# yixuan/ADMM

Measured on AMD Instinct MI355X. Metric: ADMM iterations/sec, Lasso tall n=100000 p=10000 (100-lambda warm-started path), higher is better.
Workload: dtype f32; 1 GPU; admm_lasso tall path (BASELINE configs[1]); n=100000, p=10000, nlambda=100, standardize=True, intercept=True, parallelism=single GPU, step=one cold-started warm-chained lambda path

## Files before the change

admm_amd/csrc/lasso_tall.hip:

```cpp
#include "prep.h"
#include "gemv_kernels.h"
#include "symv_kernels.h"
#include "solvers.h"
#include "sgl_host.h"
#include "box_host.h"
#include "comm.h"
#include "loop_driver.h"
#include "plan_host.h"
#include "peer_device.h"
#include "probe.h"

namespace admm {

struct TallCtl {
    double rho, lam, eps_primal, eps_dual, adj_a, adj_c, tau;
    double a_next, tau_next;
    int mode;
    int restart;
    int iter;
    int lam_idx;
    int done;
    int first;
    int total;
    int fin_idx;
    int fin_niter;
    int pad;
};

struct TallParams {
    int p, nwg, nseg, maxit, nlam, enet;
    long long part_stride;
    double eps_abs, eps_rel, alpha, sqrt_p;
    const double* lambdas;
    const float* XY;
    const float* a_part; const float* b_part;
    const float* dot0; const float* dot1; const float* axp0; const float* axp1;
    long long ldo; int nrb, p32; SymvSched sched;
    float* x; float* z0; float* z1; float* y0; float* y1; float* adj_z; float* adj_y; float* u; float* w;
    TallCtl* ctl;
    double* P;
    float* beta;
    int* niter;
    int* done_host;
#ifdef ADMM_HIP_PROBE
    long long* probe;
#endif
    double* trace;
    long long trace_cap;
    const float* refine_ab;
    long long refine_ld;
    float* state;
    long long state_cap;
    unsigned long long* verdict;
    unsigned long long run_tag;
};

__host__ __device__ inline unsigned long long tall_verdict_word(unsigned long long run_tag, int total, bool discard) {
    return run_tag | ((unsigned long long)(unsigned)total << 1) | (discard ? 1ull : 0ull);
}
constexpr int kVerdictShift = 33;
constexpr int kVerdictWords = kSyVerdictReplicas * kSyVerdictStride;

constexpr int kTailThreads = 256;
constexpr int kTailLanes = kSySumLanes;
constexpr int kTailElems = kTailThreads / kTailLanes;

__device__ __forceinline__ double tall_load_partial(const double* p, bool in_launch) {
    if (!in_launch) return *p;
    return __longlong_as_double((long long)__hip_atomic_load(reinterpret_cast<const unsigned long long*>(p), __ATOMIC_RELAXED, __HIP_MEMORY_SCOPE_AGENT));
}
__device__ __forceinline__ void tall_store_wt(float* p, float v) {
    __hip_atomic_store(reinterpret_cast<unsigned int*>(p), __float_as_uint(v), __ATOMIC_RELAXED, __HIP_MEMORY_SCOPE_AGENT);
}
__device__ __forceinline__ void tall_store_wt(double* p, double v) {
    __hip_atomic_store(reinterpret_cast<unsigned long long*>(p), (unsigned long long)__double_as_longlong(v), __ATOMIC_RELAXED, __HIP_MEMORY_SCOPE_AGENT);
}

template <bool IN_LAUNCH = false>
__device__ void tall_decide(const TallParams& q, int par) {
    __shared__ double dscratch[6 * (kTailThreads / 64)];
    WIDE_PROBE_DECL
    WIDE_PROBE(0);
    const TallCtl in = q.ctl[par];
    TallCtl* outp = &q.ctl[par ^ 1];
    if (in.done) {
        if (threadIdx.x == 0) { TallCtl o = in; o.fin_idx = -1; *outp = o; }
        return;
    }
    WIDE_PROBE(1);
    double acc[6] = {0, 0, 0, 0, 0, 0};
    const double* Pin = q.P + (size_t)par * q.nwg * 8;
    for (int w = threadIdx.x; w < q.nwg; w += kTailThreads) {
#pragma unroll
        for (int k = 0; k < 6; ++k) acc[k] += tall_load_partial(Pin + (size_t)w * 8 + k, IN_LAUNCH);
    }
    block_sum<double, 6>(acc, dscratch);
    if (threadIdx.x != 0) return;
    WIDE_PROBE(2);
    const double r2 = acc[0], dz2 = acc[1], daz2 = acc[2], x2 = acc[3], z2 = acc[4], y2 = acc[5];
    double tr_rp = 0, tr_rd = 0, tr_c = 0, tr_code = ADMM_TRACE_COLD;
    TallCtl out = in;
    out.first = 0;
    out.fin_idx = -1; out.fin_niter = 0;
    if (!in.first) {
        const double rp = sqrt(r2);
        const double rd = in.rho * sqrt(dz2);
        tr_rp = rp; tr_rd = rd;
        if (rp < in.eps_primal && rd < in.eps_dual) {
            out.fin_idx = in.lam_idx; out.fin_niter = in.iter + 1;
            out.mode = 0;
            tr_code = ADMM_TRACE_CONVERGED;
        } else {
            const double old_c = in.adj_c;
            const double c = in.rho * rp * rp + in.rho * daz2;
            tr_c = c;
            if (c < 0.999 * old_c) {
                out.adj_a = in.a_next; out.adj_c = c; out.tau = in.tau_next; out.restart = 0;
                tr_code = ADMM_TRACE_ACCELERATE;
            } else {
                out.adj_a = 1.0; out.adj_c = old_c / 0.999; out.tau = -1.0; out.restart = 1;
                tr_code = ADMM_TRACE_RESTART;
            }
            out.mode = 1;
            out.iter = in.iter + 1;
            if (in.iter + 1 >= q.maxit) {
                out.fin_idx = in.lam_idx; out.fin_niter = q.maxit + 1;
            }
        }
        if (out.fin_idx >= 0) {
            out.lam_idx = in.lam_idx + 1;
            out.iter = 0;
            if (out.lam_idx >= q.nlam) out.done = 1;
            else out.lam = q.lambdas[out.lam_idx];
            q.niter[out.fin_idx] = out.fin_niter;
        }
    } else {
        out.mode = 1; out.tau = 0.0; out.restart = 0;
    }
    if (q.verdict != nullptr && (out.mode == 0 || out.done)) {
        const unsigned long long word = tall_verdict_word(q.run_tag, in.total + 1, true);
        for (int r = 0; r < kSyVerdictReplicas; ++r)
            __hip_atomic_store(q.verdict + (size_t)r * kSyVerdictStride, word, __ATOMIC_RELAXED, __HIP_MEMORY_SCOPE_AGENT);
    }
    out.eps_primal = fmax(sqrt(x2), sqrt(z2)) * q.eps_rel + q.sqrt_p * q.eps_abs;
    out.eps_dual = sqrt(y2) * q.eps_rel + q.sqrt_p * q.eps_abs;
    out.a_next = 0.5 + 0.5 * sqrt(1.0 + 4.0 * out.adj_a * out.adj_a);
    out.tau_next = (out.adj_a - 1.0) / out.a_next;
    out.total = in.total + 1;
    *outp = out;
    if (out.done) *q.done_host = 1;
    WIDE_PROBE(3);
    WIDE_PROBE_FLUSH(2, in.total);
    if (q.trace != nullptr && in.total < q.trace_cap) {
        double* t = q.trace + (size_t)in.total * ADMM_TRACE_FIELDS;
        t[0] = in.lam_idx; t[1] = in.iter; t[2] = in.eps_primal; t[3] = in.eps_dual; t[4] = tr_rp; t[5] = tr_rd;
        t[6] = tr_c; t[7] = in.adj_c; t[8] = tr_code; t[9] = in.rho; t[10] = in.rho; t[11] = in.lam;
    }
}

struct TallDecideExtra {
    static constexpr bool kHas = true;
    TallParams q; int par;
    __device__ void operator()() const { tall_decide<false>(q, par); }
};

__device__ __forceinline__ float tall_extrapolate(float t1, float t, float cur, float old) {
#pragma clang fp contract(off)
    const float a = t1 * cur;
    const float b = t * old;
    return a - b;
}

struct TallElem { float zc, yc, zo, yo, adjz, adjy, x, xy; };

__device__ __forceinline__ TallElem tall_load_elem(const TallParams& q, int par, int i) {
    const float* zc_ = par ? q.z1 : q.z0; const float* yc_ = par ? q.y1 : q.y0;
    const float* zo_ = par ? q.z0 : q.z1; const float* yo_ = par ? q.y0 : q.y1;
    TallElem e;
    e.zc = zc_[i]; e.yc = yc_[i]; e.zo = zo_[i]; e.yo = yo_[i]; e.adjz = q.adj_z[i]; e.adjy = q.adj_y[i]; e.x = q.x[i]; e.xy = q.XY[i];
    return e;
}

__device__ __forceinline__ float tall_soft(float vec, double pen) {
    const double v = (double)vec;
    return v > pen ? (float)(v - pen) : (v < -pen ? (float)(v + pen) : 0.f);
}

__device__ __forceinline__ double tall_block_shrink(double nrm2, double pen) {
    const double nrm = sqrt(nrm2);
    return nrm > pen ? 1.0 - pen / nrm : 0.0;
}

template <bool WT = false>
__device__ __forceinline__ void tall_update_elem(const TallParams& q, const TallCtl& c, int par, int i, const TallElem& e, float a, float b, double (&acc)[6]) {
#pragma clang fp contract(off)
    float* zo_ = par ? q.z0 : q.z1; float* yo_ = par ? q.y0 : q.y1;
    const float zc = e.zc, yc = e.yc, zo = e.zo, yo = e.yo;
    if (c.fin_idx >= 0) q.beta[(size_t)c.fin_idx * q.p + i] = zc;
    if (c.done) return;
    float adjz, adjy, x;
    if (c.mode) {
        if (c.restart) { adjz = zo; adjy = yo; x = b; }
        else {
            const float t = (float)c.tau, t1 = (float)(1.0 + c.tau);
            adjz = tall_extrapolate(t1, t, zc, zo);
            adjy = tall_extrapolate(t1, t, yc, yo);
            x = a;
        }
    } else { adjz = e.adjz; adjy = e.adjy; x = e.x; }
    const float rho_f = (float)c.rho;
    const float vec = x + adjy / rho_f;
    const double pen = c.lam / c.rho;
    float zn;
    if (!q.enet) zn = tall_soft(vec, pen);
    else {
        const float thresh = (float)(q.alpha * pen);
        const float denom = (float)(1.0 + pen * (1.0 - q.alpha));
        zn = vec > thresh ? (vec - thresh) / denom : (vec < -thresh ? (vec + thresh) / denom : 0.f);
    }
    const float r = x - zn;
    const float yn = adjy + rho_f * r;
    const float dz = zn - zc, daz = zn - adjz;
    acc[0] = (double)r * r; acc[1] = (double)dz * dz; acc[2] = (double)daz * daz;
    acc[3] = (double)x * x; acc[4] = (double)zn * zn; acc[5] = (double)yn * yn;
    q.x[i] = x; zo_[i] = zn; yo_[i] = yn; q.adj_z[i] = adjz; q.adj_y[i] = adjy;
    if (q.state != nullptr && c.total < q.state_cap) {
        float* s = q.state + (size_t)c.total * 5 * q.p;
        s[i] = x; s[q.p + i] = zn; s[2 * (size_t)q.p + i] = yn; s[3 * (size_t)q.p + i] = adjz; s[4 * (size_t)q.p + i] = adjy;
    }
    const float tn = (float)c.tau_next, tn1 = (float)(1.0 + c.tau_next);
    const float adjz_a = tall_extrapolate(tn1, tn, zn, zc), adjy_a = tall_extrapolate(tn1, tn, yn, yc);
    const float un = (float)((double)(e.xy - adjy_a) + c.rho * (double)adjz_a);
    const float wn = (float)((double)(e.xy - yc) + c.rho * (double)zc);
    if (WT) { tall_store_wt(q.u + i, un); tall_store_wt(q.w + i, wn); }
    else { q.u[i] = un; q.w[i] = wn; }
}

__device__ __forceinline__ void tall_publish_norms(const TallParams& q, int par, const double (&acc)[6], double* scratch) {
    static_assert(kTailLanes == 8, "owner lanes are the multiples of 8");
    const int lane = threadIdx.x & 63, wid = threadIdx.x >> 6;
    const double v8[8] = {acc[0], acc[1], acc[2], acc[3], acc[4], acc[5], 0.0, 0.0};
    const double tot = halving_sum8_top(v8, lane);
    if ((lane & 7) == 0 && lane < 48) scratch[(lane >> 3) * (kTailThreads / 64) + wid] = tot;
    __syncthreads();
    if (threadIdx.x < 6) {
// ... 522 lines not shown
            free_b += pool_cached_bytes();
            if (opt_set(Opt::TEST_FREE_BYTES)) free_b = (size_t)opt_int(Opt::TEST_FREE_BYTES, 0);
            const bool have_gram = d.gram.get() && d.ldgram == ldp;
            const bool inv64_wanted = p < 4096 || opt_is(Opt::INVERSE, "f64");
            const double mat = (double)ldp * (double)ldp * 4.0;
            const double need = (have_gram ? 0.0 : mat) + (inv64_wanted ? 2.0 * mat : 0.5 * mat) + (opt_on(Opt::REFINE) ? mat : 0.0) +
                                (shard && ci.nranks > 1 ? mat + mat / ci.nranks : 0.0) +
                                (mt ? mt_partial_floats() * 4.0 : 0.0);
            if (need > 0.97 * (double)free_b) {
                char msg[320];
                std::snprintf(msg, sizeof msg, "tall solver: the cached %d x %d inverse and its workspace need %.1f GB, the device has %.1f GB free; "
                              "use $parallel() (row blocks, admm_hip_parlasso) or fewer columns", p, p, need / 1e9, (double)free_b / 1e9);
                throw Error(ADMM_ERR_MEMORY, msg);
            }
        }
        double t0 = now_s();
        const bool gram_given = d.gram.get() && d.ldgram == ldp;
        if (gram_given) {
            M = std::move(d.gram);
            S.t_gram = d.t_gram_tail;
        } else {
            M.alloc((size_t)ldp * ldp); M.zero(st);
            gram_full<float>(d.X.get(), d.ldx, n, p, true, M.get(), ldp, st);
            comm_stream_sync(st);
            S.t_gram = now_s() - t0;
        }
        bool inv64 = p < 4096;
        if (opt_set(Opt::INVERSE)) inv64 = opt_is(Opt::INVERSE, "f64");
        bool dist_factor = shard && ci.nranks > 1 && !inv64 && (p + 127) / 128 >= 2 * ci.nranks && p >= 256;
        if (opt_off(Opt::DIST_FACTOR)) dist_factor = false;

        rho = pb.opts.rho;
        t0 = now_s();
        if (rho <= 0) {
            SymMatVec<float> op(M.get(), ldp, p, st);
            int nmatop = 0;
            DevBuf<float> wsum;
            if (shard && ci.nranks > 1) wsum.alloc(ldp);
            const float ev = lanczos_largest_f32([&](const float* v, float* w_) {
                op(v, w_);
                if (shard && ci.nranks > 1) {
                    ADMM_HIP_CHECK(hipMemcpyAsync(wsum.get(), w_, (size_t)p * sizeof(float), hipMemcpyHostToDevice, st));
                    allreduce_sum_f32(wsum.get(), (size_t)p, st);
                    ADMM_HIP_CHECK(hipMemcpyAsync(w_, wsum.get(), (size_t)p * sizeof(float), hipMemcpyDeviceToHost, st));
                    comm_stream_sync(st);
                    comm_check();
                }
            }, p, &nmatop);
            S.eig_est = ev;
            rho = std::pow((double)ev, 1.0 / 3) * std::pow(lam_int[0], 2.0 / 3);
        }
        S.rho = rho;
        S.t_eigs = now_s() - t0;

        if (shard && ci.nranks > 1 && !gram_given) {
            const double tr0 = now_s();
            if (dist_factor) {
                const int nb128 = (p + 127) / 128, N = ci.nranks;
                const int nown = (nb128 + N - 1) / N;
                const size_t blk = (size_t)128 * ldp, cnt = (size_t)nown * blk;
                DevBuf<float> send((size_t)N * cnt), recv(cnt);
                send.zero(st);
                for (int k = 0; k < nb128; ++k) {
                    const size_t cols = (size_t)std::min(128, (int)ldp - k * 128);
                    ADMM_HIP_CHECK(hipMemcpyAsync(send.get() + ((size_t)(k % N) * nown + k / N) * blk, M.get() + (size_t)k * blk, cols * ldp * sizeof(float),
                                                  hipMemcpyDeviceToDevice, st));
                }
                reduce_scatter_sum_f32(send.get(), recv.get(), cnt, st);
                for (int k = ci.rank; k < nb128; k += N) {
                    const size_t cols = (size_t)std::min(128, (int)ldp - k * 128);
                    ADMM_HIP_CHECK(hipMemcpyAsync(M.get() + (size_t)k * blk, recv.get() + (size_t)(k / N) * blk, cols * ldp * sizeof(float), hipMemcpyDeviceToDevice, st));
                }
            } else {
                allreduce_sum_f32(M.get(), (size_t)ldp * ldp, st);
            }
            comm_stream_sync(st);
            comm_check();
            S.t_gram += now_s() - tr0;
        }

        refine = opt_on(Opt::REFINE) && !shard;
        if (refine) {
            Mg.alloc((size_t)ldp * ldp);
            ADMM_HIP_CHECK(hipMemcpyAsync(Mg.get(), M.get(), (size_t)ldp * ldp * sizeof(float), hipMemcpyDeviceToDevice, st));
            add_diag<float>(Mg.get(), ldp, p, (float)rho, st);
        }
        t0 = now_s();
        if (inv64) {
            spd_inverse_f32_via_f64(M.get(), ldp, p, (double)(float)rho, st);
        } else if (dist_factor) {
            add_diag<float>(M.get(), ldp, p, (float)rho, st);
            sy.init(p, st, ci.rank, ci.nranks);
            std::vector<int> need;
            {
                const int nb128 = (p + 127) / 128;
                std::vector<char> mark((size_t)nb128 * nb128, 0);
                for (const int4& t : sy.htiles)
                    for (int bi = 2 * t.x; bi <= 2 * t.x + 1 && bi < nb128; ++bi)
                        for (int bj = t.y / 128; bj <= (t.y + t.z - 1) / 128 && bj < nb128; ++bj)
                            if (bj <= bi && !mark[(size_t)bi * nb128 + bj]) { mark[(size_t)bi * nb128 + bj] = 1; need.push_back(bi << 16 | bj); }
            }
            double fl = 0;
            spd_inverse_mfma_f32_dist(M.get(), ldp, p, need, &fl, st);
            dist_flops = fl;
        } else {
            add_diag<float>(M.get(), ldp, p, (float)rho, st);
            spd_inverse_f32(M.get(), ldp, p, st);
        }
        comm_stream_sync(st);
        S.t_factor = now_s() - t0;
        d.X.release();

        use_sym = p >= 2048;
        if (opt_set(Opt::XUPDATE)) use_sym = opt_is(Opt::XUPDATE, "sym");
        if (refine) use_sym = true;
        if (shard) use_sym = true;
        if (mt) use_sym = true;
        pl = plan_gemv_t<float>(p, p, 2, 4);
        nwg = (p + kTailElems - 1) / kTailElems;
        if (grouped) nwg = pack_group_tiles();
        ldv = round_up(p, 256);
        if (use_sym) sy.init(p, st, shard ? ci.rank : 0, shard ? ci.nranks : 1);
        if (refine) {
            rab.alloc((size_t)2 * ldv); rab.zero(st);
            ruw.alloc((size_t)2 * ldv); ruw.zero(st);
            dD0.alloc((size_t)sy.nrb * sy.ldo); dD1.alloc((size_t)sy.nrb * sy.ldo);
            xD0.alloc((size_t)sy.nax_rows * sy.ldo); xD1.alloc((size_t)sy.nax_rows * sy.ldo);
            dD0.zero(st); dD1.zero(st); xD0.zero(st); xD1.zero(st);
        }
        if (shard) { ab.alloc((size_t)2 * ldp); ab.zero(st); }
        else if (!use_sym) { a_part.alloc((size_t)pl.nseg * ldp); b_part.alloc((size_t)pl.nseg * ldp); a_part.zero(st); b_part.zero(st); }
        const ExchangeForm xf = peer_exchange_form(shard, ci, reinterpret_cast<const void*>(tall_tail_kernel<TAIL_PEER1>), kTailThreads, nwg);
        peer_fused = xf.fused; peer_one = xf.one; exchange_code = xf.variant;
        const size_t npl = (size_t)std::max(mt, 1);
        x.alloc(npl * ldv); z0.alloc(npl * ldv); z1.alloc(npl * ldv); y0.alloc(npl * ldv); y1.alloc(npl * ldv);
        adj_z.alloc(npl * ldv); adj_y.alloc(npl * ldv); u.alloc(ldv); w.alloc(ldv);
        beta.alloc((size_t)nlam * p * npl); niter.alloc(nlam);
        P.alloc((size_t)2 * nwg * 8); dlam.alloc(nlam); ctl.alloc(2);
        u.zero(st); w.zero(st);
        ADMM_HIP_CHECK(hipMemcpyAsync(dlam.get(), lam_int.data(), nlam * sizeof(double), hipMemcpyHostToDevice, st));

        q.p = p; q.nwg = nwg; q.nseg = pl.nseg; q.maxit = pb.opts.maxit; q.nlam = nlam; q.enet = pb.enet ? 1 : 0;
        q.part_stride = ldp;
        q.eps_abs = pb.opts.eps_abs; q.eps_rel = pb.opts.eps_rel; q.alpha = (double)(float)pb.alpha; q.sqrt_p = std::sqrt((double)p * (double)npl);
        q.lambdas = dlam.get(); q.XY = XY.get(); q.a_part = a_part.get(); q.b_part = b_part.get();
        if (shard) { q.a_part = ab.get(); q.b_part = ab.get() + ldp; q.nseg = 1; }
        q.dot0 = sy.dot0.get(); q.dot1 = sy.dot1.get(); q.axp0 = sy.axp0.get(); q.axp1 = sy.axp1.get();
        q.ldo = sy.ldo; q.nrb = sy.nrb; q.p32 = sy.p32; q.sched = sy.sched;
        q.refine_ab = refine ? rab.get() : nullptr; q.refine_ld = ldv;
        q.x = x.get(); q.z0 = z0.get(); q.z1 = z1.get(); q.y0 = y0.get(); q.y1 = y1.get();
        q.adj_z = adj_z.get(); q.adj_y = adj_y.get(); q.u = u.get(); q.w = w.get();
        q.ctl = ctl.get(); q.P = P.get(); q.beta = beta.get(); q.niter = niter.get();
        q.done_host = hflag.p;
        verdict_on = use_sym && !shard && !refine && !mt && !opt_off(Opt::SYMV_VERDICT);
        verdict_mid = opt_int(Opt::SYMV_VERDICT, 2) == 2;
        if (verdict_on) {
            verdict.alloc(kVerdictWords + kSyVerdictStride); verdict.zero(st);
            q.verdict = verdict.get();
        }
#ifdef ADMM_HIP_PROBE
        probe.alloc((size_t)4096 * 4 * 8); probe.zero(st);
        q.probe = probe.get();
        sy.probe = probe.get();
#endif

        if (mt) {
            static const int kAutoRhs[kMtMax] = {2, 4, 8, 8, 12, 12, 8, 8, 4, 4, 12, 12, 4, 4, 8, 8};
            mt_rhs = kAutoRhs[mt - 1];
            if (const OptValue* v = opt(Opt::MT_RHS)) { if (v->i > 0) mt_rhs = kSyNR[v->i - 1]; }
            uw.alloc((size_t)2 * mt * ldv); uw.zero(st);
            const size_t ds = (size_t)sy.nrb * sy.ldo, as = (size_t)sy.nax_rows * sy.ldo;
            mdot.alloc((size_t)2 * mt * ds); maxp.alloc((size_t)2 * mt * as);
            mdot.zero(st); maxp.zero(st);
            x.zero(st); z0.zero(st); z1.zero(st); y0.zero(st); y1.zero(st); adj_z.zero(st); adj_y.zero(st);
            roww.alloc(p);
            ADMM_HIP_CHECK(hipMemcpyAsync(roww.get(), pb.row_weight.data(), (size_t)p * sizeof(double), hipMemcpyHostToDevice, st));
            mq.m = mt; mq.ldv = ldv; mq.ldxy = ldp; mq.uw = uw.get();
            mq.dot = mdot.get(); mq.axp = maxp.get(); mq.dot_stride = (long long)ds; mq.axp_stride = (long long)as;
            mq.row_w = roww.get();
        }
        ADMM_HIP_CHECK(hipHostMalloc(reinterpret_cast<void**>(&hbeta), (size_t)nlam * p * npl * sizeof(float), hipHostMallocDefault));
        comm_stream_sync(st);
    }

    float box_plan_lambda0() {
        std::vector<float> lo(p), hi(p), h(p);
        for (int j = 0; j < p; ++j) {
            lo[j] = box_round_lower(box_to_std(pb.box_lower[j], (double)d.scaleX[j], (double)d.scaleY));
            hi[j] = box_round_upper(box_to_std(pb.box_upper[j], (double)d.scaleX[j], (double)d.scaleY));
        }
        clamp.set(pb.box_lower, pb.box_upper);
        bpf.alloc((size_t)p); blo.alloc((size_t)p); bhi.alloc((size_t)p);
        ADMM_HIP_CHECK(hipMemcpyAsync(bpf.get(), pb.penalty_factor.data(), (size_t)p * sizeof(double), hipMemcpyHostToDevice, st));
        ADMM_HIP_CHECK(hipMemcpyAsync(blo.get(), lo.data(), (size_t)p * sizeof(float), hipMemcpyHostToDevice, st));
        ADMM_HIP_CHECK(hipMemcpyAsync(bhi.get(), hi.data(), (size_t)p * sizeof(float), hipMemcpyHostToDevice, st));
        read_back(h.data(), XY.get(), (size_t)p * sizeof(float), st);
        bq.pf = bpf.get(); bq.lo = blo.get(); bq.hi = bhi.get();
        return box_lambda0(h.data(), p, lo.data(), hi.data(), pb.penalty_factor.data());
    }

    float mt_lambda0() {
        std::vector<float> h((size_t)mt * ldp);
        read_back(h.data(), XY.get(), h.size() * sizeof(float), st);
        double best = 0.0;
        for (int j = 0; j < p; ++j) {
            if (!(pb.row_weight[j] > 0)) continue;
            double s2 = 0.0;
            for (int k = 0; k < mt; ++k) { const double v = (double)h[(size_t)k * ldp + j]; s2 += v * v; }
            best = std::max(best, std::sqrt(s2) / pb.row_weight[j]);
        }
        return (float)best;
    }
    double mt_partial_floats() const {
        const double nrb = (double)((p + kSyRB - 1) / kSyRB), ldo = nrb * kSyRB;
        return 2.0 * mt * (nrb + (double)((p + 31) / 32)) * ldo;
    }

    float group_lambda0() {
        std::vector<float> h(p);
        read_back(h.data(), XY.get(), (size_t)p * sizeof(float), st);
        double best = 0.0;
        for (size_t g = 0; g + 1 < pb.group_start.size(); ++g) {
            if (!(pb.group_weight[g] > 0)) continue;
            double s2 = 0.0;
            for (int j = pb.group_start[g]; j < pb.group_start[g + 1]; ++j) s2 += (double)h[j] * (double)h[j];
            best = std::max(best, std::sqrt(s2) / pb.group_weight[g]);
        }
        return (float)best;
    }

    float sgl_plan_lambda0() {
        std::vector<float> h(p);
        read_back(h.data(), XY.get(), (size_t)p * sizeof(float), st);
        return sgl_lambda0(h.data(), pb.group_start, pb.l1_weight, pb.group_weight);
    }

    int pack_group_tiles() {
        std::vector<int2> tiles;
        std::vector<GroupCoord> coord(p);
        const bool flat = pb.sgl && std::none_of(pb.group_weight.begin(), pb.group_weight.end(), [](double w) { return w > 0; });
        std::vector<int> each;
        if (flat) for (int j = 0; j <= p; ++j) each.push_back(j);
        const std::vector<int>& start = flat ? each : pb.group_start;
        int first = 0, count = 0;
        const auto flush = [&] { if (count > 0) tiles.push_back(make_int2(first, count)); first += count; count = 0; };
        for (size_t g = 0; g + 1 < start.size(); ++g) {
            const int gs = start[g], gn = start[g + 1] - gs;
            const double wg = flat ? 0.0 : pb.group_weight[g];
            ADMM_REQUIRE(gn >= 1 && gn <= kGroupMax && gs == first + count, "internal: bad group partition");
            for (int j = gs; j < gs + gn; ++j)
                coord[j] = GroupCoord{gs, gn, pb.sgl && gn == 1 ? sgl_single_weight(pb.l1_weight[j], wg) : wg};
            if (count + gn > kTailElems) flush();
            count += gn;
            if (gn > kTailElems) flush();
        }
        flush();
        gtiles.alloc(tiles.size()); gcoord.alloc(coord.size());
        ADMM_HIP_CHECK(hipMemcpyAsync(gtiles.get(), tiles.data(), tiles.size() * sizeof(int2), hipMemcpyHostToDevice, st));
        ADMM_HIP_CHECK(hipMemcpyAsync(gcoord.get(), coord.data(), coord.size() * sizeof(GroupCoord), hipMemcpyHostToDevice, st));
        if (pb.sgl) {
            gl1.alloc((size_t)p);
            ADMM_HIP_CHECK(hipMemcpyAsync(gl1.get(), pb.l1_weight.data(), (size_t)p * sizeof(double), hipMemcpyHostToDevice, st));
        }
        comm_stream_sync(st);
        gq.tiles = gtiles.get(); gq.coord = gcoord.get(); gq.l1 = pb.sgl ? gl1.get() : nullptr;
        return (int)tiles.size();
    }

    Records records() override { return {st, 5ll * p * std::max(mt, 1), &q.trace, &q.trace_cap, &q.state, &q.state_cap}; }

    void read_system(float* out, long long ld) override {
        if (!refine) throw Error(ADMM_ERR_INVALID_ARG, "the system matrix is only kept with ADMM_HIP_REFINE=1");
        ADMM_REQUIRE(out != nullptr && ld >= p, "bad output for the system matrix");
        ADMM_HIP_CHECK(hipMemcpy2D(out, (size_t)ld * sizeof(float), Mg.get(), (size_t)ldp * sizeof(float), (size_t)p * sizeof(float), (size_t)p, hipMemcpyDeviceToHost));
    }

    void run(LassoResult& res) override {
        admm_stats S = setup_stats;
        S.xupdate_variant = shard ? 2 : (use_sym ? 1 : 0);
        S.exchange_variant = exchange_code;
        S.refine = refine ? 1 : 0;
        S.factor_flops = dist_flops;
        res.lambda = lam_user;
        beta.zero(st); niter.zero(st);
        q.run_tag = ++run_no << kVerdictShift;
        const int init_n = std::max(p, 2 * nwg * 8);
        for (int k = 0; k < std::max(mt, 1); ++k) {
            TallParams qk = q;
            if (mt) {
                const size_t o = (size_t)k * ldv;
                qk.x += o; qk.z0 += o; qk.z1 += o; qk.y0 += o; qk.y1 += o; qk.adj_z += o; qk.adj_y += o;
                qk.XY += (size_t)k * ldp; qk.u = uw.get() + (size_t)(2 * k) * ldv; qk.w = uw.get() + (size_t)(2 * k + 1) * ldv;
            }
            hipLaunchKernelGGL(tall_init_kernel, dim3((init_n + 255) / 256), dim3(256), 0, st, qk, rho, lam_int[0]);
        }
        if (q.state != nullptr && mt)
            ADMM_HIP_CHECK(hipMemcpy2DAsync(q.state, (size_t)p * sizeof(float), XY.get(), (size_t)ldp * sizeof(float), (size_t)p * sizeof(float),
                                            (size_t)mt, hipMemcpyDeviceToDevice, st));
        else if (q.state != nullptr)
            ADMM_HIP_CHECK(hipMemcpyAsync(q.state, XY.get(), (size_t)p * sizeof(float), hipMemcpyDeviceToDevice, st));
        *hflag.p = 0;
#ifdef ADMM_HIP_PROBE
        sy.probe_idx = 0;
#endif

        const int batch = batch_iters(pb.batch_iters, 32);
        const int stride = pb.profile_stride;
        size_t nev = 0;
        const auto done_at = [&](long long g) -> const int* { return &ctl.get()[(int)(g & 1)].done; };
        const LoopTimes lt = run_until_done(st, done_at, batch, (long long)nlam * ((long long)pb.opts.maxit + 2) + 4, [&](long long g) {
            const int par = (int)(g & 1);
            const bool sample = stride > 0 && (g % stride) == stride / 2 && nev < 8192;
            hipEvent_t e0 = nullptr, e1 = nullptr;
            if (sample) {
                while (ev_pool.size() < nev + 2) {
                    hipEvent_t e; ADMM_HIP_CHECK(hipEventCreate(&e));
                    ev_pool.push_back(e);
                }
                e0 = ev_pool[nev]; e1 = ev_pool[nev + 1];
                nev += 2;
            }
            const TallDecideExtra dec{q, par};
            SymvVerdict vd;
            if (verdict_on) { vd.words = verdict.get(); vd.discard = tall_verdict_word(q.run_tag, (int)(g + 1), true); vd.early = verdict.get() + kVerdictWords; vd.mid = verdict_mid; }
            const int* skip = &ctl.get()[par].done;
            const auto xupdate = [&] {
                if (use_sym) sy.launch(M.get(), ldp, u.get(), w.get(), skip, st, dec, e0, e1, vd);
                else launch_gemv_t<float, 2, 4, TallDecideExtra>(pl, M.get(), ldp, p, p, u.get(), w.get(), a_part.get(), b_part.get(), ldp, skip, st, dec, e0, e1);
            };
            const auto group_tail = [&] {
                void (*tail)(TallParams, int, GroupTailParams) =
                    use_sym ? (pb.sgl ? tall_group_tail_kernel<TAIL_SYMV, true> : tall_group_tail_kernel<TAIL_SYMV>)
                            : (pb.sgl ? tall_group_tail_kernel<TAIL_GEMV, true> : tall_group_tail_kernel<TAIL_GEMV>);
                hipLaunchKernelGGL(tail, dim3(nwg), dim3(kTailThreads), 0, st, q, par, gq);
            };
            if (mt) {
                const int nvec = 2 * mt;
                for (int r0 = 0; r0 < nvec; r0 += mt_rhs) {
                    SymvNArgs a;
                    a.A = M.get(); a.lda = ldp; a.p = p;
                    a.v = uw.get() + (size_t)r0 * ldv; a.vstride = ldv;
                    a.dot = mdot.get() + (size_t)r0 * mq.dot_stride; a.dot_stride = mq.dot_stride;
                    a.axp = maxp.get() + (size_t)r0 * mq.axp_stride; a.axp_stride = mq.axp_stride;
                    a.nvec = std::min(mt_rhs, nvec - r0); a.ldo = sy.ldo; a.tiles = sy.tiles.get(); a.skip = skip;
                    hipEvent_t es = r0 == 0 ? e0 : nullptr, ee = r0 + mt_rhs >= nvec ? e1 : nullptr;
                    if (r0 == 0) symvn_launch(sy, mt_rhs, a, st, dec, es, ee);
                    else symvn_launch(sy, mt_rhs, a, st, SymvNoExtra(), es, ee);
                }
                hipLaunchKernelGGL(tall_mt_tail_kernel, dim3(nwg), dim3(kTailThreads), 0, st, q, par, mq);
            } else if (grouped) {
                xupdate();
                group_tail();
            } else if (shard && peer_fused) {
                sy.launch(M.get(), ldp, u.get(), w.get(), skip, st, dec, e0, e1);
                const PeerExchange ex = comm_peer_begin((size_t)2 * ldp * sizeof(float));
                if (peer_one) {
                    hipLaunchKernelGGL(tall_tail_kernel<TAIL_PEER1>, dim3(nwg), dim3(kTailThreads), 0, st, q, par, ex);
                } else {
                    hipLaunchKernelGGL(tall_shard_push_kernel, dim3(nwg), dim3(kTailThreads), 0, st, q, ex, ldp, skip);
                    hipLaunchKernelGGL(tall_tail_kernel<TAIL_PEER>, dim3(nwg), dim3(kTailThreads), 0, st, q, par, ex);
                }
            } else if (shard) {
                sy.launch(M.get(), ldp, u.get(), w.get(), skip, st, dec, e0, e1);
                hipLaunchKernelGGL(tall_shard_reduce_kernel, dim3(nwg), dim3(kTailThreads), 0, st, q, ab.get(), ldp, skip);
                allreduce_sum_f32(ab.get(), (size_t)2 * ldp, st);
                hipLaunchKernelGGL(tall_tail_kernel<TAIL_GEMV>, dim3(nwg), dim3(kTailThreads), 0, st, q, par, PeerExchange{});
            } else if (use_sym && refine) {
                sy.launch(M.get(), ldp, u.get(), w.get(), skip, st, dec, e0, e1);
                hipLaunchKernelGGL(tall_shard_reduce_kernel, dim3(nwg), dim3(kTailThreads), 0, st, q, rab.get(), ldv, skip);
                SymvArgsD ad;
                ad.A = Mg.get(); ad.lda = ldp; ad.p = p; ad.v0 = rab.get(); ad.v1 = rab.get() + ldv;
                ad.dot0 = dD0.get(); ad.dot1 = dD1.get(); ad.axp0 = xD0.get(); ad.axp1 = xD1.get(); ad.ldo = sy.ldo; ad.tiles = sy.tiles.get(); ad.skip = skip;
                hipLaunchKernelGGL(symv2_lower_f64acc_kernel, dim3(sy.ntiles), dim3(kSyThreads), 0, st, ad);
                hipLaunchKernelGGL(tall_refine_resid_kernel, dim3(nwg), dim3(kTailThreads), 0, st, q, dD0.get(), dD1.get(), xD0.get(), xD1.get(),
                                   ruw.get(), ruw.get() + ldv, skip);
                sy.launch(M.get(), ldp, ruw.get(), ruw.get() + ldv, skip, st, SymvNoExtra());
                hipLaunchKernelGGL(tall_tail_kernel<TAIL_SYMV>, dim3(nwg), dim3(kTailThreads), 0, st, q, par, PeerExchange{});
            } else if (pb.box) {
                xupdate();
                if (use_sym) hipLaunchKernelGGL(tall_box_tail_kernel<TAIL_SYMV>, dim3(nwg), dim3(kTailThreads), 0, st, q, par, bq);
                else hipLaunchKernelGGL(tall_box_tail_kernel<TAIL_GEMV>, dim3(nwg), dim3(kTailThreads), 0, st, q, par, bq);
            } else {
                xupdate();
                if (use_sym) hipLaunchKernelGGL(tall_tail_kernel<TAIL_SYMV>, dim3(nwg), dim3(kTailThreads), 0, st, q, par, PeerExchange{});
                else hipLaunchKernelGGL(tall_tail_kernel<TAIL_GEMV>, dim3(nwg), dim3(kTailThreads), 0, st, q, par, PeerExchange{});
            }
        }, LoopOpts{shard ? nullptr : hflag.p, 0, false});
        S.t_loop = lt.wall_s; S.loop_ms_events = lt.events_ms; S.xupdate_launches = lt.launched;
        const CtlPair<TallCtl> hctl = read_ctl(ctl.get());
        unsigned long long early = 0;
        if (verdict_on) ADMM_HIP_CHECK(hipMemcpy(&early, verdict.get() + kVerdictWords, sizeof early, hipMemcpyDeviceToHost));
        t_early_exits = (long long)early;
        WIDE_PROBE_DUMP(probe);
        if (nev > 0) {
            double tot = 0;
            for (size_t k = 0; k + 1 < nev; k += 2) {
                float m1 = 0.f;
                ADMM_HIP_CHECK(hipEventElapsedTime(&m1, ev_pool[k], ev_pool[k + 1]));
                tot += m1;
            }
            S.xupdate_samples = (long long)(nev / 2);
            S.xupdate_ms_avg = tot / (double)(nev / 2);
        }

        ADMM_HIP_CHECK(hipMemcpyAsync(hbeta, beta.get(), (size_t)nlam * p * std::max(mt, 1) * sizeof(float), hipMemcpyDeviceToHost, st));
        comm_stream_sync(st);
        if (mt) {
            const size_t col = (size_t)p + 1;
            std::vector<float> bk;
            res.beta.assign(col * mt * nlam, 0.f);
            for (int k = 0; k < mt; ++k) {
                S.total_iter = read_out_path<float>(d, hbeta + (size_t)k * p, nlam, niter.get(), col, 0, res.niter, bk, INT_MAX, (size_t)mt * p, &d.meanYs[k]);
                for (int l = 0; l < nlam; ++l) std::memcpy(res.beta.data() + ((size_t)l * mt + k) * col, bk.data() + (size_t)l * col, col * sizeof(float));
            }
        } else {
            S.total_iter = read_out_path<float>(d, hbeta, nlam, niter.get(), (size_t)p + 1, 0, res.niter, res.beta, INT_MAX, 0, nullptr, &clamp);
        }
        decisions = hctl.c[0].done ? hctl.total() : 0;
        res.stats = S;
    }
};

std::unique_ptr<LassoPlan> make_tall_plan(DeviceData<float>&& d, const LassoProblem& pb, hipStream_t st) {
    return std::unique_ptr<LassoPlan>(new TallPlan(std::move(d), pb, st));
}

}
```

admm_amd/csrc/options.h:

```cpp
#pragma once
#include <limits>
#include <string>
#include <vector>

namespace admm {

enum class OptKind { Flag, Int, Real, Choice, Text, Sched, Devices };
struct OptAccepts {
    OptKind kind;
    double lo = 0, hi = 0;
    const char* choices = nullptr;
};
constexpr OptAccepts Flag() { return {OptKind::Flag, 0, 1}; }
constexpr OptAccepts Int(double lo, double hi) { return {OptKind::Int, lo, hi}; }
constexpr OptAccepts Real(double lo, double hi) { return {OptKind::Real, lo, hi}; }
constexpr OptAccepts Choice(const char* c) { return {OptKind::Choice, 0, 0, c}; }
constexpr OptAccepts Text() { return {OptKind::Text}; }
constexpr OptAccepts Sched() { return {OptKind::Sched}; }
constexpr OptAccepts Devices() { return {OptKind::Devices}; }
constexpr double kPositive = std::numeric_limits<double>::min();

#define ADMM_OPTIONS(X)                                                                                                                  \
    X(BATCH_ITERS, Int(1, 1 << 20), "iterations enqueued between two host polls (rounded up to even; default per solver)")             \
    X(PROFILE_STRIDE, Int(0, 1 << 30), "time every k-th tall x-update launch with HIP events (0: off)")                                 \
    X(GRAM, Choice("rocblas|oneshot"), "tall Gram through rocBLAS / host input transferred before the Gram is built")                    \
    X(GRAM_SPLIT, Choice("0|f16x2|bf16x3"), "tall Gram of order >= ~4000: exact fp32 kernel / fp16 x 2 (default) / bf16 x 3")          \
    X(GRAM_B3_KTILES, Int(0, 1 << 20), "K tiles per launch of the 16-bit split Gram (0: one launch)")                                   \
    X(FACTOR, Choice("rocsolver"), "Cholesky + inverse through rocSOLVER / rocBLAS instead of the hand-written kernels")                \
    X(INVERSE, Choice("f32|f64"), "precision the cached inverse is built in")                                                           \
    X(XUPDATE, Choice("sym|gemv|full"), "tall x-update: symmetric lower-triangle kernel / full-matrix mat-vec (gemv and full alike)")   \
    X(SYMV_SCHED, Sched(), "tall x-update: column-segment widths of the long / short row strips and the split between them")           \
    X(SYMV_VERDICT, Choice("0|1|2"), "tall x-update: tiles of a discarded launch leave never / when they start / also mid-tile (default)") \
    X(REFINE, Flag(), "tall path: refine every x-update with a double-precision residual")                                               \
    X(DIST_FACTOR, Flag(), "row-sharded tall solver: 0 = every rank factorises the whole all-reduced Gram")                            \
    X(CV_DOWNDATE, Flag(), "cross-validation folds' Grams as down-dates of the full-data Gram: 1 always, 0 never")                      \
    X(PREP_FUSED, Flag(), "0: convert, column statistics and standardisation as separate sweeps over X")                                \
    X(H2D, Choice("pageable"), "host inputs through plain hipMemcpy instead of the pinned staging ring")                                 \
    X(POOL_MB, Int(0, 1 << 30), "cache of released device blocks, megabytes (0: off)")                                                  \
    X(WIDE_FUSE, Flag(), "wide path: 0 = three launches per iteration")                                                                  \
    X(WIDE_TGLOBAL, Flag(), "wide path: 1 = t through global memory instead of LDS")                                                     \
    X(WIDE_SPRAD, Choice("gram"), "wide path: spectral radius from the explicit n x n Gram")                                            \
    X(WIDE_SCREEN, Choice("0|8|16|auto"), "wide path: screen the regular steps never / 8-bit code / fp16 copy / chosen at any size")    \
    X(WIDE_SCREEN_STATS, Flag(), "wide path: print the screen's counts")                                                                 \
    X(WIDE_PERSIST, Flag(), "wide path: 0 = no persistent active-set stretches")                                                         \
    X(WIDE_PERSIST_COLS, Flag(), "column-sharded wide solver: 0 = no persistent active-set stretches")                                  \
    X(WIDE_ROWS_C, Int(1, 32), "wide path: column groups of the 2-D stretch (kept only when it fits with the problem's row groups)")    \
    X(WIDE_PERSIST_STATS, Flag(), "wide path: print the stretch statistics")                                                             \
    X(PAR_ONEPASS, Flag(), "consensus solver: 0 = the reference's two products per Woodbury worker")                                    \
    X(PAR_ONEPASS_TAU, Real(0, 1e300), "one-pass Woodbury workers: threshold of the cancellation guard (0: never fall back)")           \
    X(PAR_ONEPASS_STATS, Flag(), "one-pass Woodbury workers: print how many worker-iterations took the dense pass")                     \
    X(PAR_FUSE_PZ, Flag(), "consensus solver: 0 = pack and z as two launches")                                                           \
    X(PAR_BATCH, Flag(), "consensus solver: 0 = one launch per worker and product")                                                      \
    X(PAR_DEVICES, Devices(), "admm_hip_parlasso / admm_hip_parbp over several devices in one process")                                \
    X(TEST_PAR_FAIL_RANK, Int(0, 63), "test hook: this rank of an in-process call fails before its first exchange")                    \
    X(PEER_FUSED, Choice("0|1|2"), "PEER back-end: 0 = the generic all-reduce, 2 = producer and consumer as two launches")             \
    X(PEER_MEM, Choice("uncached"), "PEER exchange buffers as uncached device memory")                                                   \
    X(COMM_SLOT_BYTES, Int(4096, 1ll << 40), "payload capacity of one PEER / SHM exchange (rounded down to 16 bytes)")                 \
    X(COMM_TIMEOUT_S, Real(kPositive, 1e300), "wait bound of the per-iteration exchanges, seconds")                                    \
    X(COMM_PATIENT_TIMEOUT_S, Real(kPositive, 1e300), "wait bound of setup reductions and replica joins, seconds")                     \
    X(LAD_HAT, Flag(), "LAD: 0 = the general projection also for n <= 2000")                                                            \
    X(LAD_ONEPASS, Flag(), "LAD: 0 = the reference's two products per iteration")                                                      \
    X(QUANT_SLOTS, Int(0, 8), "admm_hip_quantreg: quantiles per pass over X on the one-pass branch: 0 = automatic, 1 = serial, else at most that many") \
    X(MT_RHS, Choice("0|2|4|8|12"), "admm_hip_mtlasso: right-hand sides per pass over the cached inverse (0: automatic)")               \
    X(BP_ONEPASS, Flag(), "basis pursuit: 0 = the reference's two products per iteration")                                             \
    X(SBP_GRAM, Flag(), "admm_hip_parbp: 0 = the direct launches on every active-set iteration")                                       \
    X(SBP_GRAM_CAP, Int(1, 1024), "admm_hip_parbp: most columns of the Gram-space matrix (rounded to multiples of 8)")                 \
    X(SBP_GRAM_CARRY, Flag(), "admm_hip_parbp: 0 = every Gram-space stretch starts from the direct launches' n-vectors")              \
    X(SBP_SCREEN, Flag(), "admm_hip_parbp: screen the regular iterations always / never")                                             \
    X(SBP_SCREEN_STATS, Flag(), "admm_hip_parbp: print the screen's counts")                                                           \
    X(SBP_WGS, Int(1, 1 << 20), "admm_hip_parbp: workgroups of the x-update launches")                                                 \
    X(SBP_SHARE, Int(1, 1 << 20), "admm_hip_parbp: smallest share of a block's non-zero list a workgroup takes")                      \
    X(SBP_TEST_DELAY_US, Int(0, 1000000), "test hook: every even workgroup of a Gram-space launch starts that many us late")           \
    X(TEST_RESIDENT_WGS, Int(0, 1ll << 40), "test hook: pretend the device holds that many resident workgroups")                      \
    X(TEST_FREE_BYTES, Int(0, 1ll << 52), "test hook: pretend the device has that many bytes free")                                    \
    X(PROBE_OUT, Text(), "dev build with in-kernel timestamps (-DADMM_HIP_PROBE): file the probe records go to")

enum class Opt : int {
#define ADMM_OPT_ID(id, accepts, summary) id,
    ADMM_OPTIONS(ADMM_OPT_ID)
#undef ADMM_OPT_ID
};
constexpr int kNumOptions = 0
#define ADMM_OPT_COUNT(id, accepts, summary) +1
    ADMM_OPTIONS(ADMM_OPT_COUNT)
#undef ADMM_OPT_COUNT
    ;

struct OptValue {
    std::string text;
    long long i = 0;
    double r = 0;
    int sched[3] = {0, 0, 0};
};
struct ThreadOptions {
    bool has[kNumOptions] = {};
    OptValue v[kNumOptions];
};

const OptValue* opt(Opt id);
inline bool opt_set(Opt id) { return opt(id) != nullptr; }
inline long long opt_int(Opt id, long long dflt) { const OptValue* v = opt(id); return v ? v->i : dflt; }
inline double opt_real(Opt id, double dflt) { const OptValue* v = opt(id); return v ? v->r : dflt; }
inline const char* opt_text(Opt id) { const OptValue* v = opt(id); return v ? v->text.c_str() : nullptr; }
inline bool opt_on(Opt id) { return opt_int(id, -1) == 1; }
inline bool opt_off(Opt id) { return opt_int(id, -1) == 0; }
bool opt_is(Opt id, const char* choice);

inline int batch_iters(int set, int dflt) { return set > 0 ? (set + 1) / 2 * 2 : dflt; }

bool opt_find(const char* name, Opt* id);
void opt_parse(Opt id, const char* text, OptValue* out);
ThreadOptions& thread_options();
void opt_set_thread(Opt id, const char* value);
void check_option_overlay();
std::vector<int> parse_par_devices(const char* v, int device_count);

}
```

admm_amd/csrc/plan_host.h:

```cpp
#pragma once
#include "solvers.h"
#include "comm.h"
#include "box_host.h"
#include <climits>

namespace admm {

template <typename Round, typename Stored>
int make_path_grid(const LassoProblem& pb, double lambda0, long long n, double scaleY, std::vector<double>& user, std::vector<Stored>& internal) {
    user = make_lambda_grid(pb, lambda0, (int)n, scaleY);
    internal.resize(user.size());
    for (size_t i = 0; i < user.size(); ++i) internal[i] = (Stored)(Round)(user[i] * (double)n / scaleY);
    return (int)user.size();
}

template <typename T>
long long read_out_path(const DeviceData<T>& d, const T* snap, int nlam, const int* dev_niter, size_t stride, long long col_offset,
                        std::vector<int>& niter, std::vector<T>& beta, int niter_clip = INT_MAX, size_t snap_stride = 0,
                        const T* mean_y = nullptr, const BoxClamp* box = nullptr) {
    if (snap_stride == 0) snap_stride = (size_t)d.p;
    niter.assign(nlam, 0);
    ADMM_HIP_CHECK(hipMemcpy(niter.data(), dev_niter, (size_t)nlam * sizeof(int), hipMemcpyDeviceToHost));
    beta.assign(stride * nlam, T(0));
    long long tot = 0;
    for (int l = 0; l < nlam; ++l) {
        T b0 = 0;
        T* out = beta.data() + (size_t)l * stride + 1 + col_offset;
        recover_coef<T>(d, mean_y ? *mean_y : d.meanY, snap + (size_t)l * snap_stride, &b0, out);
        if (box != nullptr && box->on() && box->apply(out, d.p) && (d.flag & 2)) {
            T acc = T(0);
            for (int j = 0; j < d.p; ++j) acc += out[j] * d.meanX[j];
            b0 = (mean_y ? *mean_y : d.meanY) - acc;
        }
        beta[(size_t)l * stride] = b0;
        tot += std::min(niter[l], niter_clip);
    }
    return tot;
}

template <typename Ctl>
struct CtlPair {
    Ctl c[2];
    long long total() const { return std::max(c[0].total, c[1].total); }
    const Ctl& finished() const { return c[0].done ? c[0] : c[1]; }
};
template <typename Ctl>
CtlPair<Ctl> read_ctl(const Ctl* dev) {
    CtlPair<Ctl> h;
    ADMM_HIP_CHECK(hipMemcpy(h.c, dev, sizeof(h.c), hipMemcpyDeviceToHost));
    return h;
}

inline int exchange_variant(bool sharded, bool fused, bool one) { return !sharded ? 0 : (!fused ? 1 : (one ? 3 : 2)); }

struct ExchangeForm { bool fused = false, one = false; int variant = 0; };
inline ExchangeForm peer_exchange_form(bool sharded, const CommInfo& ci, const void* one_kernel, int block, long long grid) {
    ExchangeForm f;
    f.fused = sharded && ci.backend == COMM_PEER && !opt_is(Opt::PEER_FUSED, "0");
    if (f.fused) {
        int occ = 0;
        ADMM_HIP_CHECK(hipOccupancyMaxActiveBlocksPerMultiprocessor(&occ, one_kernel, block, 0));
        f.one = grid * 2 <= resident_workgroups(occ) && !opt_is(Opt::PEER_FUSED, "2");
    }
    f.variant = exchange_variant(sharded, f.fused, f.one);
    return f;
}

}
```

Measured before the change: 26430 iterations/s.

## Prefetch decision partials before control read, batch readout copies, parallelize coefficient recovery

The decision tail now issues loads of the first two rounds of per-workgroup norm partials before reading the control block, at raised wave priority, so the two memory latencies overlap. After the loop, the beta snapshot, the control pair and the early-exit counter are copied asynchronously into one pinned buffer with a single stream sync, replacing separate blocking copies. Coefficient recovery on the host is split across up to 8 threads and can write directly into a caller-provided destination. In exchange the tail carries extra register pressure, and the host side adds thread creation cost and relies on new beta_dst/beta_written result fields.

```diff
diff --git a/admm_amd/csrc/lasso_tall.hip b/admm_amd/csrc/lasso_tall.hip
--- a/admm_amd/csrc/lasso_tall.hip
+++ b/admm_amd/csrc/lasso_tall.hip
@@ -53,6 +53,7 @@
     long long state_cap;
     unsigned long long* verdict;
     unsigned long long run_tag;
+    int decide_early;
 };
 
 __host__ __device__ inline unsigned long long tall_verdict_word(unsigned long long run_tag, int total, bool discard) {
@@ -60,6 +61,9 @@
 }
 constexpr int kVerdictShift = 33;
 constexpr int kVerdictWords = kSyVerdictReplicas * kSyVerdictStride;
+
+struct TallReadOut { CtlPair<TallCtl> ctl; unsigned long long early; };
+inline size_t tall_readout_offset(size_t nbeta_floats) { return (nbeta_floats + 3) / 4 * 4; }
 
 constexpr int kTailThreads = 256;
 constexpr int kTailLanes = kSySumLanes;
@@ -75,22 +79,57 @@
 __device__ __forceinline__ void tall_store_wt(double* p, double v) {
     __hip_atomic_store(reinterpret_cast<unsigned long long*>(p), (unsigned long long)__double_as_longlong(v), __ATOMIC_RELAXED, __HIP_MEMORY_SCOPE_AGENT);
 }
+
+__device__ __forceinline__ void tall_pin(double v) { asm volatile("" :: "v"(v)); }
+constexpr int kDecidePre = 2;
 
 template <bool IN_LAUNCH = false>
 __device__ void tall_decide(const TallParams& q, int par) {
     __shared__ double dscratch[6 * (kTailThreads / 64)];
     WIDE_PROBE_DECL
     WIDE_PROBE(0);
-    const TallCtl in = q.ctl[par];
     TallCtl* outp = &q.ctl[par ^ 1];
-    if (in.done) {
-        if (threadIdx.x == 0) { TallCtl o = in; o.fin_idx = -1; *outp = o; }
-        return;
-    }
-    WIDE_PROBE(1);
+    const double* Pin = q.P + (size_t)par * q.nwg * 8;
     double acc[6] = {0, 0, 0, 0, 0, 0};
-    const double* Pin = q.P + (size_t)par * q.nwg * 8;
-    for (int w = threadIdx.x; w < q.nwg; w += kTailThreads) {
+    int wnext = threadIdx.x;
+    TallCtl in;
+    if (q.decide_early) {
+        __builtin_amdgcn_s_setprio(3);
+        double pre[kDecidePre][6];
+#pragma unroll
+        for (int j = 0; j < kDecidePre; ++j) {
+            const int w = min((int)threadIdx.x + j * kTailThreads, q.nwg - 1);
+#pragma unroll
+            for (int k = 0; k < 6; ++k) pre[j][k] = tall_load_partial(Pin + (size_t)w * 8 + k, IN_LAUNCH);
+        }
+        in = q.ctl[par];
+#pragma unroll
+        for (int j = 0; j < kDecidePre; ++j) {
+#pragma unroll
+            for (int k = 0; k < 6; ++k) tall_pin(pre[j][k]);
+        }
+        if (in.done) {
+            if (threadIdx.x == 0) { TallCtl o = in; o.fin_idx = -1; *outp = o; }
+            return;
+        }
+        WIDE_PROBE(1);
+#pragma unroll
+        for (int j = 0; j < kDecidePre; ++j) {
+            if ((int)threadIdx.x + j * kTailThreads < q.nwg) {
+#pragma unroll
+                for (int k = 0; k < 6; ++k) acc[k] += pre[j][k];
+            }
+        }
+        wnext += kDecidePre * kTailThreads;
+    } else {
+        in = q.ctl[par];
+        if (in.done) {
+            if (threadIdx.x == 0) { TallCtl o = in; o.fin_idx = -1; *outp = o; }
+            return;
+        }
+        WIDE_PROBE(1);
+    }
+    for (int w = wnext; w < q.nwg; w += kTailThreads) {
 #pragma unroll
         for (int k = 0; k < 6; ++k) acc[k] += tall_load_partial(Pin + (size_t)w * 8 + k, IN_LAUNCH);
     }
@@ -919,6 +958,7 @@
         q.adj_z = adj_z.get(); q.adj_y = adj_y.get(); q.u = u.get(); q.w = w.get();
         q.ctl = ctl.get(); q.P = P.get(); q.beta = beta.get(); q.niter = niter.get();
         q.done_host = hflag.p;
+        q.decide_early = opt_off(Opt::TALL_DECIDE_EARLY) ? 0 : 1;
         verdict_on = use_sym && !shard && !refine && !mt && !opt_off(Opt::SYMV_VERDICT);
         verdict_mid = opt_int(Opt::SYMV_VERDICT, 2) == 2;
         if (verdict_on) {
@@ -946,7 +986,7 @@
             mq.dot = mdot.get(); mq.axp = maxp.get(); mq.dot_stride = (long long)ds; mq.axp_stride = (long long)as;
             mq.row_w = roww.get();
         }
-        ADMM_HIP_CHECK(hipHostMalloc(reinterpret_cast<void**>(&hbeta), (size_t)nlam * p * npl * sizeof(float), hipHostMallocDefault));
+        ADMM_HIP_CHECK(hipHostMalloc(reinterpret_cast<void**>(&hbeta), tall_readout_offset((size_t)nlam * p * npl) * sizeof(float) + sizeof(TallReadOut), hipHostMallocDefault));
         comm_stream_sync(st);
     }
 
@@ -1154,10 +1194,15 @@
             }
         }, LoopOpts{shard ? nullptr : hflag.p, 0, false});
         S.t_loop = lt.wall_s; S.loop_ms_events = lt.events_ms; S.xupdate_launches = lt.launched;
-        const CtlPair<TallCtl> hctl = read_ctl(ctl.get());
-        unsigned long long early = 0;
-        if (verdict_on) ADMM_HIP_CHECK(hipMemcpy(&early, verdict.get() + kVerdictWords, sizeof early, hipMemcpyDeviceToHost));
-        t_early_exits = (long long)early;
+        const size_t nbeta = (size_t)nlam * p * std::max(mt, 1);
+        TallReadOut* const ho = reinterpret_cast<TallReadOut*>(hbeta + tall_readout_offset(nbeta));
+        ho->early = 0;
+        ADMM_HIP_CHECK(hipMemcpyAsync(hbeta, beta.get(), nbeta * sizeof(float), hipMemcpyDeviceToHost, st));
+        ADMM_HIP_CHECK(hipMemcpyAsync(ho->ctl.c, ctl.get(), sizeof(ho->ctl.c), hipMemcpyDeviceToHost, st));
+        if (verdict_on) ADMM_HIP_CHECK(hipMemcpyAsync(&ho->early, verdict.get() + kVerdictWords, sizeof ho->early, hipMemcpyDeviceToHost, st));
+        comm_stream_sync(st);
+        const CtlPair<TallCtl> hctl = ho->ctl;
+        t_early_exits = (long long)ho->early;
         WIDE_PROBE_DUMP(probe);
         if (nev > 0) {
             double tot = 0;
@@ -1170,8 +1215,6 @@
             S.xupdate_ms_avg = tot / (double)(nev / 2);
         }
 
-        ADMM_HIP_CHECK(hipMemcpyAsync(hbeta, beta.get(), (size_t)nlam * p * std::max(mt, 1) * sizeof(float), hipMemcpyDeviceToHost, st));
-        comm_stream_sync(st);
         if (mt) {
             const size_t col = (size_t)p + 1;
             std::vector<float> bk;
@@ -1181,7 +1224,8 @@
                 for (int l = 0; l < nlam; ++l) std::memcpy(res.beta.data() + ((size_t)l * mt + k) * col, bk.data() + (size_t)l * col, col * sizeof(float));
             }
         } else {
-            S.total_iter = read_out_path<float>(d, hbeta, nlam, niter.get(), (size_t)p + 1, 0, res.niter, res.beta, INT_MAX, 0, nullptr, &clamp);
+            S.total_iter = read_out_path<float>(d, hbeta, nlam, niter.get(), (size_t)p + 1, 0, res.niter, res.beta, INT_MAX, 0, nullptr, &clamp, res.beta_dst);
+            res.beta_written = res.beta_dst != nullptr;
         }
         decisions = hctl.c[0].done ? hctl.total() : 0;
         res.stats = S;
diff --git a/admm_amd/csrc/options.h b/admm_amd/csrc/options.h
--- a/admm_amd/csrc/options.h
+++ b/admm_amd/csrc/options.h
@@ -31,6 +31,8 @@
     X(XUPDATE, Choice("sym|gemv|full"), "tall x-update: symmetric lower-triangle kernel / full-matrix mat-vec (gemv and full alike)")   \
     X(SYMV_SCHED, Sched(), "tall x-update: column-segment widths of the long / short row strips and the split between them")           \
     X(SYMV_VERDICT, Choice("0|1|2"), "tall x-update: tiles of a discarded launch leave never / when they start / also mid-tile (default)") \
+    X(TALL_DECIDE_EARLY, Flag(), "tall path: 0 = the decision asks for the norm partials only after it has read its control block")        \
+    X(READOUT_THREADS, Int(1, 64), "host threads that recover the coefficient columns of a finished path (1: serial; default up to 8)")    \
     X(REFINE, Flag(), "tall path: refine every x-update with a double-precision residual")                                               \
     X(DIST_FACTOR, Flag(), "row-sharded tall solver: 0 = every rank factorises the whole all-reduced Gram")                            \
     X(CV_DOWNDATE, Flag(), "cross-validation folds' Grams as down-dates of the full-data Gram: 1 always, 0 never")                      \
diff --git a/admm_amd/csrc/plan_host.h b/admm_amd/csrc/plan_host.h
--- a/admm_amd/csrc/plan_host.h
+++ b/admm_amd/csrc/plan_host.h
@@ -3,6 +3,8 @@
 #include "comm.h"
 #include "box_host.h"
 #include <climits>
+#include <system_error>
+#include <thread>
 
 namespace admm {
 
@@ -14,27 +16,53 @@
     return (int)user.size();
 }
 
+constexpr long long kReadOutPerThread = 1ll << 17;
+inline int read_out_threads(int nlam, long long p) {
+    const unsigned hw = std::thread::hardware_concurrency();
+    long long nt = std::min<long long>(8, (long long)nlam * p / kReadOutPerThread);
+    if (const OptValue* v = opt(Opt::READOUT_THREADS)) nt = v->i;
+    nt = std::min<long long>(nt, std::max(1u, hw));
+    return (int)std::max(1ll, std::min<long long>(nt, nlam));
+}
+
 template <typename T>
 long long read_out_path(const DeviceData<T>& d, const T* snap, int nlam, const int* dev_niter, size_t stride, long long col_offset,
                         std::vector<int>& niter, std::vector<T>& beta, int niter_clip = INT_MAX, size_t snap_stride = 0,
-                        const T* mean_y = nullptr, const BoxClamp* box = nullptr) {
+                        const T* mean_y = nullptr, const BoxClamp* box = nullptr, T* dst = nullptr) {
     if (snap_stride == 0) snap_stride = (size_t)d.p;
     niter.assign(nlam, 0);
     ADMM_HIP_CHECK(hipMemcpy(niter.data(), dev_niter, (size_t)nlam * sizeof(int), hipMemcpyDeviceToHost));
-    beta.assign(stride * nlam, T(0));
+    if (dst == nullptr) { beta.assign(stride * nlam, T(0)); dst = beta.data(); }
+    else {
+        beta.clear();
+        if (col_offset != 0 || stride != (size_t)d.p + 1) std::fill(dst, dst + stride * nlam, T(0));
+    }
+    const auto columns = [&](int l0, int l1) {
+        for (int l = l0; l < l1; ++l) {
+            T b0 = 0;
+            T* out = dst + (size_t)l * stride + 1 + col_offset;
+            recover_coef<T>(d, mean_y ? *mean_y : d.meanY, snap + (size_t)l * snap_stride, &b0, out);
+            if (box != nullptr && box->on() && box->apply(out, d.p) && (d.flag & 2)) {
+                T acc = T(0);
+                for (int j = 0; j < d.p; ++j) acc += out[j] * d.meanX[j];
+                b0 = (mean_y ? *mean_y : d.meanY) - acc;
+            }
+            dst[(size_t)l * stride] = b0;
+        }
+    };
+    const int nt = read_out_threads(nlam, d.p);
+    const auto first = [&](int t) { return (int)((long long)nlam * t / nt); };
+    std::vector<std::thread> workers;
+    workers.reserve((size_t)nt);
+    int started = 1;
+    try {
+        for (; started < nt; ++started) workers.emplace_back(columns, first(started), first(started + 1));
+    } catch (const std::system_error&) {}
+    columns(0, first(1));
+    columns(first(started), nlam);
+    for (std::thread& w : workers) w.join();
     long long tot = 0;
-    for (int l = 0; l < nlam; ++l) {
-        T b0 = 0;
-        T* out = beta.data() + (size_t)l * stride + 1 + col_offset;
-        recover_coef<T>(d, mean_y ? *mean_y : d.meanY, snap + (size_t)l * snap_stride, &b0, out);
-        if (box != nullptr && box->on() && box->apply(out, d.p) && (d.flag & 2)) {
-            T acc = T(0);
-            for (int j = 0; j < d.p; ++j) acc += out[j] * d.meanX[j];
-            b0 = (mean_y ? *mean_y : d.meanY) - acc;
-        }
-        beta[(size_t)l * stride] = b0;
-        tot += std::min(niter[l], niter_clip);
-    }
+    for (int l = 0; l < nlam; ++l) tot += std::min(niter[l], niter_clip);
     return tot;
 }
 
```

Result: no change. 26350 iterations/s (-0.3%).
